# alanross/AlvaAR

Measured on NVIDIA H100. Metric: frames_per_sec_720p_1000orb_20kf_ba, higher is better.
Workload: dtype u8/f64

## Files before the change

alvaar_b200/csrc/ba.cu:

```cuda
#include "alva_common.cuh"
#include "../../include/alva_b200.h"
#include <math.h>
#include <float.h>
#include <string.h>

namespace {

constexpr int NMAX = 128;
constexpr int LIN_THREADS = 128;
constexpr int NBMAX = NMAX / 6;
constexpr int MAXKEYS = NBMAX * (NBMAX + 1) / 2;
constexpr int BS_THREADS = 128;

struct BaState {
    double radius, decrease_factor, x_cost, cand_cost, xnorm, gmax, model_change;
    double se_min, se_cur, se_ref, se_cand, se_acc_ref, se_acc_cand;
    double initial_cost, push_cost;
    int reuse_diagonal, invalid_steps, iteration, last_success, n_success, n_iter, term, done;
    int relin, step_ok, ncols, chol_ok;
    int use_gather, nb, nbad, has_last;
    int skipped, pad0;
};

struct BaProblem {
// ... 143 lines not shown
__device__ __forceinline__ double block_sum(double v, double* sm) {
    sm[threadIdx.x] = v;
    __syncthreads();
    for (int s = NT / 2; s > 0; s >>= 1) {
        if ((int)threadIdx.x < s) sm[threadIdx.x] += sm[threadIdx.x + s];
        __syncthreads();
    }
    return sm[0];
}

__device__ __forceinline__ double block_sum_dyn(double v, double* sm) {
#pragma unroll
    for (int off = 16; off; off >>= 1) v += __shfl_xor_sync(0xffffffffu, v, off);
    const int lane = threadIdx.x & 31, warp = threadIdx.x >> 5, nw = (blockDim.x + 31) >> 5;
    __syncthreads();
    if (lane == 0) sm[warp] = v;
    __syncthreads();
    if (threadIdx.x == 0) { double t = 0; for (int w = 0; w < nw; w++) t += sm[w]; sm[32] = t; }
    __syncthreads();
    return sm[32];
}
__device__ __forceinline__ double block_max_dyn(double v, double* sm) {
#pragma unroll
    for (int off = 16; off; off >>= 1) v = fmax(v, __shfl_xor_sync(0xffffffffu, v, off));
    const int lane = threadIdx.x & 31, warp = threadIdx.x >> 5, nw = (blockDim.x + 31) >> 5;
    __syncthreads();
    if (lane == 0) sm[warp] = v;
    __syncthreads();
    if (threadIdx.x == 0) { double t = sm[0]; for (int w = 1; w < nw; w++) t = fmax(t, sm[w]); sm[32] = t; }
    __syncthreads();
    return sm[32];
}

constexpr int SETUP_THREADS = 1024;
__global__ void __launch_bounds__(SETUP_THREADS) ba_setup_kernel(const BaProblem* __restrict__ probs, BaDims D) {
    const BaProblem P = probs[blockIdx.x];
    if (threadIdx.x < NBMAX) P.ga_ticket[threadIdx.x] = 0;
    __shared__ int ref[256];
    __shared__ int scan_s[SETUP_THREADS + 1];
    __shared__ int wcount[32][NBMAX + 1];
    __shared__ int run[NBMAX + 1], pl_base[NBMAX + 1];
    const int tid = threadIdx.x, lane = tid & 31, warp = tid >> 5;
    constexpr int NT = SETUP_THREADS;
    if (D.pass == 1 && (P.st->nbad == 0 || !(D.huber > 0))) {
        if (tid == 0) { P.st->done = 1; P.st->skipped = 1; P.st->use_gather = 0; P.st->has_last = 0; }
        return;
    }
    for (int k = tid; k < 256; k += NT) ref[k] = 0;
    for (int l = tid; l <= D.nlm; l += NT) P.lm_start[l] = 0;
    __syncthreads();
    for (int o = tid; o < D.nobs; o += NT) {
        const int l = P.obs_lm[o];
        if (l < 0) continue;
        atomicAdd(&P.lm_start[l + 1], 1);
        ref[P.anch_kf[l]] = 1;
        ref[P.obs_kf[o]] = 1;
    }
    __syncthreads();
    if (tid == 0) {
        int c = 0;
        for (int k = 0; k < D.nkf; k++) {
            if (!P.pose_const[k] && ref[k]) { P.pose_col[k] = c; c += 6; }
            else P.pose_col[k] = -1;
        }
        BaState& s = *P.st;
        s.ncols = c;
// ... 89 lines not shown
    maxobs = max(maxobs, __shfl_xor_sync(0xffffffffu, maxobs, 4)); maxobs = max(maxobs, __shfl_xor_sync(0xffffffffu, maxobs, 2));
    maxobs = max(maxobs, __shfl_xor_sync(0xffffffffu, maxobs, 1));
    if (lane == 0) scan_s[warp] = maxobs;
    __syncthreads();
    if (tid == 0) {
        int mo = 0;
        for (int i = 0; i < NT / 32; i++) mo = max(mo, scan_s[i]);
        P.st->use_gather = (mo < 255 && D.nlm < 65536 && D.nobs < 65535) ? 1 : 0;
    }
}

template <bool FULL>
__device__ __forceinline__ double lin_obs(const BaProblem& P, const BaDims& D, int o, int l, const double* poses, double invd_l) {
    const int ka = P.anch_kf[l], kp = P.obs_kf[o];
    double r[2], Ja[12], Jp[12], Jd[2];
    ba_evaluate(P.calib, poses + 7 * ka, poses + 7 * kp, invd_l, P.obs_uv[2 * o], P.obs_uv[2 * o + 1], P.anch_uv[2 * l],
                P.anch_uv[2 * l + 1], r, FULL ? Ja : nullptr, Jp, Jd);
    double rho0, rho1;
    huber(r[0] * r[0] + r[1] * r[1], D.huber, rho0, rho1);
    if (FULL) {
        const double sc = sqrt(rho1);
        r[0] *= sc; r[1] *= sc;
        P.res[2 * o] = r[0]; P.res[2 * o + 1] = r[1];
        Jd[0] *= sc; Jd[1] *= sc;
        P.Jd[2 * o] = Jd[0]; P.Jd[2 * o + 1] = Jd[1];
#pragma unroll
        for (int i = 0; i < 12; i++) { Ja[i] *= sc; Jp[i] *= sc; P.Ja[12 * o + i] = Ja[i]; P.Jp[12 * o + i] = Jp[i]; }
    }
    return 0.5 * rho0;
}

template <bool FULL>
__global__ void __launch_bounds__(LIN_THREADS, 7) ba_linearize_kernel(const BaProblem* __restrict__ probs, BaDims D) {
    const BaProblem P = probs[blockIdx.y];
    __shared__ double red[LIN_THREADS];
    const BaState& st = *P.st;
    const bool active = FULL ? (st.relin && !st.done) : !st.done;
    if (!active) return;
    const int o = blockIdx.x * LIN_THREADS + threadIdx.x;
    double cost = 0;
    const int l = o < D.nobs ? P.obs_lm[o] : -1;
    if (l >= 0) cost = lin_obs<FULL>(P, D, o, l, FULL ? P.poses : P.cand_poses, (FULL ? P.invd : P.cand_invd)[l]);
    const double tot = block_sum<LIN_THREADS>(cost, red);
    if (threadIdx.x == 0) P.cost_part[blockIdx.x] = tot;
}

__device__ __forceinline__ void stats_landmark(const BaProblem& P, int l) {
    double ne = 0, ge = 0;
    for (int i = P.lm_start[l]; i < P.lm_start[l + 1]; i++) {
        const int o = P.lm_obs[i];
        const double d0 = P.Jd[2 * o], d1 = P.Jd[2 * o + 1];
        ne += d0 * d0 + d1 * d1;
        ge += d0 * P.res[2 * o] + d1 * P.res[2 * o + 1];
    }
    P.ne[l] = ne;
    P.ge[l] = ge;
}
__device__ __forceinline__ void stats_pose_partial(const BaProblem& P, int b, int gt, double* v) {
    int eb = 0;
    for (int i = 0; i < b; i++) eb += P.pstart[i + 1];
    const int ee = eb + P.pstart[b + 1];
#pragma unroll
    for (int i = 0; i < 12; i++) v[i] = 0;
    for (int idx = eb + gt; idx < ee; idx += BS_THREADS) {
        const uint32_t en = P.plist[idx];
        const int l = en >> 8, su = en & 0xff;
        const int ob = P.lm_start[l];
        if (su) {
            const int o = P.lm_obs[ob + su - 1];
            const double r0 = P.res[2 * o], r1 = P.res[2 * o + 1];
#pragma unroll
            for (int c = 0; c < 6; c++) {
                const double j0 = P.Jp[12 * o + c], j1 = P.Jp[12 * o + 6 + c];
                v[c] += j0 * j0 + j1 * j1;
                v[6 + c] += j0 * r0 + j1 * r1;
            }
        } else {
            for (int i = ob; i < P.lm_start[l + 1]; i++) {
                const int o = P.lm_obs[i];
                const double r0 = P.res[2 * o], r1 = P.res[2 * o + 1];
#pragma unroll
                for (int c = 0; c < 6; c++) {
                    const double j0 = P.Ja[12 * o + c], j1 = P.Ja[12 * o + 6 + c];
                    v[c] += j0 * j0 + j1 * j1;
                    v[6 + c] += j0 * r0 + j1 * r1;
                }
            }
        }
    }
}

__global__ void __launch_bounds__(BS_THREADS) ba_stats_kernel(const BaProblem* __restrict__ probs, BaDims D) {
    const BaProblem P = probs[blockIdx.y];
    const BaState& st = *P.st;
    if (st.done || !st.relin) return;
    __shared__ double part[4][12];
    if ((int)blockIdx.x < D.nbs) {
        const int l = blockIdx.x * BS_THREADS + threadIdx.x;
        if (l >= D.nlm) return;
        stats_landmark(P, l);
        return;
    }
    const int b = blockIdx.x - D.nbs;
    if (b >= st.ncols / 6) return;
    const int lane = threadIdx.x & 31, warp = threadIdx.x >> 5;
    double v[12];
    stats_pose_partial(P, b, threadIdx.x, v);
#pragma unroll
    for (int i = 0; i < 12; i++) {
#pragma unroll
        for (int off = 16; off; off >>= 1) v[i] += __shfl_xor_sync(0xffffffffu, v[i], off);
        if (lane == 0) part[warp][i] = v[i];
    }
    __syncthreads();
    if (threadIdx.x < 12) {
        const double t = part[0][threadIdx.x] + part[1][threadIdx.x] + part[2][threadIdx.x] + part[3][threadIdx.x];
        if (threadIdx.x < 6) P.nf[6 * b + threadIdx.x] = t;
        else P.gf[6 * b + threadIdx.x - 6] = t;
    }
}

template <int MODE>
__global__ void __launch_bounds__(32) ba_pairs_kernel(const BaProblem* __restrict__ probs, BaDims D) {
    const BaProblem P = probs[blockIdx.y];
    BaState& st = *P.st;
// ... 122 lines not shown
    __syncthreads();
    if (tid == 0) {
        if (st.last_success) st.n_success++;
        st.n_iter++;
        int cont = 1;
        if (st.iteration >= D.max_iter) { st.term = 1; cont = 0; }
        else if (st.last_success && st.gmax <= 1e-10) { st.term = 0; cont = 0; }
        else if (st.radius <= 1e-32) { st.term = 0; cont = 0; }
        if (!cont) st.done = 1;
        else { st.iteration++; st.last_success = 0; }
        go = cont;
    }
    __syncthreads();
    if (!go) return;
    const bool reuse = st.reuse_diagonal;
    const double radius = st.radius;
    __syncthreads();
    for (int i = tid; i < n; i += NT) {
        if (!reuse) P.diagf[i] = fmin(fmax(P.nf[i] * P.scf[i] * P.scf[i], 1e-6), 1e32);
        P.Df[i] = sqrt(P.diagf[i] / radius);
    }
    for (int l = tid; l < D.nlm; l += NT) {
        if (!reuse) P.diage[l] = fmin(fmax(P.ne[l] * P.sce[l] * P.sce[l], 1e-6), 1e32);
        P.De[l] = sqrt(P.diage[l] / radius);
    }
    for (int i = tid; i < NMAX * NMAX; i += NT) P.S[i] = 0;
    for (int i = tid; i < NMAX; i += NT) P.rhs[i] = 0;
    __syncthreads();
    for (int i = tid; i < n; i += NT) P.S[i * NMAX + i] = P.Df[i] * P.Df[i];
    if (tid == 0) st.reuse_diagonal = 1;
}

__global__ void __launch_bounds__(CT_THREADS) ba_pre_kernel(const BaProblem* __restrict__ probs, BaDims D) {
    const BaProblem P = probs[blockIdx.x];
    ba_pre_body(P, D);
}

template <bool DENSE>
__device__ void schur_landmark(const BaProblem& P, const BaDims& D, int l) {
    if (DENSE) {
        double* row = P.Wt + (size_t)l * NMAX;
        for (int i = 0; i < NMAX; i++) row[i] = 0.0;
    }
    if (l >= D.nlm) return;
    const int b = P.lm_start[l], e = P.lm_start[l + 1];
    if (e == b) return;
    const int ca = P.pose_col[P.anch_kf[l]];
    const double sce = P.sce[l];
    double ete = P.De[l] * P.De[l], etb = 0, wa[6] = {0, 0, 0, 0, 0, 0};
    double sca[6];
    for (int c = 0; c < 6; c++) sca[c] = ca >= 0 ? P.scf[ca + c] : 0.0;
    double Saa[36];
    for (int i = 0; i < 36; i++) Saa[i] = 0;
    double rha[6] = {0, 0, 0, 0, 0, 0};
    for (int i = b; i < e; i++) {
        const int o = P.lm_obs[i];
        const int cp = P.pose_col[P.obs_kf[o]];
        const double e0 = P.Jd[2 * o] * sce, e1 = P.Jd[2 * o + 1] * sce;
        const double r0 = P.res[2 * o], r1 = P.res[2 * o + 1];
        ete += e0 * e0 + e1 * e1;
        etb += e0 * r0 + e1 * r1;
        double Fa[12], Fp[12];
        for (int c = 0; c < 6; c++) {
            Fa[c] = P.Ja[12 * o + c] * sca[c]; Fa[6 + c] = P.Ja[12 * o + 6 + c] * sca[c];
            const double s = cp >= 0 ? P.scf[cp + c] : 0.0;
            Fp[c] = P.Jp[12 * o + c] * s; Fp[6 + c] = P.Jp[12 * o + 6 + c] * s;
// ... 41 lines not shown
            for (int c = 0; c < 6; c++) {
                row[ci + c] += P.wp[6 * oi + c] * rs;
                atomicAdd(&P.rhs[ci + c], -P.wp[6 * oi + c] * inv * etb);
            }
        }
        return;
    }
    for (int i = b; i < e; i++) {
        const int oi = P.lm_obs[i];
        const int ci = P.pose_col[P.obs_kf[oi]];
        if (ci < 0) continue;
        double wi[6];
        for (int c = 0; c < 6; c++) wi[c] = P.wp[6 * oi + c];
        for (int a = 0; a < 6; a++) atomicAdd(&P.rhs[ci + a], -wi[a] * inv * etb);
        if (ca >= 0)
            for (int a = 0; a < 6; a++)
                for (int c = 0; c < 6; c++) {
                    const double x = -wa[a] * inv * wi[c];
                    atomicAdd(&P.S[(ca + a) * NMAX + ci + c], x);
                    atomicAdd(&P.S[(ci + c) * NMAX + ca + a], x);
                }
        for (int j = b; j < e; j++) {
            const int oj = P.lm_obs[j];
            const int cj = P.pose_col[P.obs_kf[oj]];
            if (cj < 0) continue;
            for (int a = 0; a < 6; a++)
                for (int c = 0; c < 6; c++) atomicAdd(&P.S[(ci + a) * NMAX + cj + c], -wi[a] * inv * P.wp[6 * oj + c]);
        }
    }
}

template <bool DENSE>
__global__ void __launch_bounds__(128) ba_schur_kernel(const BaProblem* __restrict__ probs, BaDims D) {
    const BaProblem P = probs[blockIdx.y];
    if (P.st->done) return;
    if (!DENSE && P.st->use_gather) return;
    const int l = blockIdx.x * 128 + threadIdx.x;
    if (l >= D.nlm_pad) return;
    schur_landmark<DENSE>(P, D, l);
}

__device__ __forceinline__ void dmma_m8n8k4(double& c0, double& c1, double a, double b) {
    asm volatile("mma.sync.aligned.m8n8k4.row.col.f64.f64.f64.f64 {%0, %1}, {%2}, {%3}, {%0, %1};"
                 : "+d"(c0), "+d"(c1)
                 : "d"(a), "d"(b));
}

constexpr int SYRK_KSPLIT = 8;

__global__ void __launch_bounds__(128) ba_syrk_dmma_kernel(const BaProblem* __restrict__ probs, BaDims D) {
    const BaProblem P = probs[blockIdx.z];
    if (P.st->done) return;
    __shared__ double part[4][32][33];
    const int lane = threadIdx.x & 31, warp = threadIdx.x >> 5;
    const int bi = blockIdx.x >> 2, bj = blockIdx.x & 3;
    const int i0 = bi * 32, j0 = bj * 32;
    const int n = P.st->ncols;
    if (i0 >= n || j0 >= n) return;
    const int ksteps = D.nlm_pad / 4;
    const int per = (ksteps + SYRK_KSPLIT - 1) / SYRK_KSPLIT;
    const int kb = blockIdx.y * per, ke = min(ksteps, kb + per);
    double acc[4][4][2];
#pragma unroll
    for (int a = 0; a < 4; a++)
#pragma unroll
        for (int b = 0; b < 4; b++) acc[a][b][0] = acc[a][b][1] = 0.0;
    const int kr = lane & 3, cc = lane >> 2;
    for (int ks = kb + warp; ks < ke; ks += 4) {
        const double* row = P.Wt + (size_t)(4 * ks + kr) * NMAX;
        double av[4], bv[4];
#pragma unroll
        for (int t = 0; t < 4; t++) { av[t] = __ldg(row + i0 + 8 * t + cc); bv[t] = __ldg(row + j0 + 8 * t + cc); }
#pragma unroll
        for (int a = 0; a < 4; a++)
#pragma unroll
            for (int b = 0; b < 4; b++) dmma_m8n8k4(acc[a][b][0], acc[a][b][1], av[a], bv[b]);
    }
#pragma unroll
    for (int a = 0; a < 4; a++)
#pragma unroll
        for (int b = 0; b < 4; b++) {
            part[warp][8 * a + cc][8 * b + 2 * kr] = acc[a][b][0];
            part[warp][8 * a + cc][8 * b + 2 * kr + 1] = acc[a][b][1];
        }
    __syncthreads();
    for (int t = threadIdx.x; t < 32 * 32; t += 128) {
        const int r = t >> 5, c = t & 31;
        const double v = part[0][r][c] + part[1][r][c] + part[2][r][c] + part[3][r][c];
        if (v != 0.0) atomicAdd(&P.S[(i0 + r) * NMAX + j0 + c], -v);
    }
}


__device__ __forceinline__ void lm_landmark(const BaProblem& P, int l) {
    const int b = P.lm_start[l], e = P.lm_start[l + 1];
    if (e == b) return;
    const int ca = P.pose_col[P.anch_kf[l]];
    const double sce = P.sce[l];
    double ete = P.De[l] * P.De[l], etb = 0, wa[6] = {0, 0, 0, 0, 0, 0};
    for (int i = b; i < e; i++) {
        const int o = P.lm_obs[i];
        const int cp = P.pose_col[P.obs_kf[o]];
        const double e0 = P.Jd[2 * o] * sce, e1 = P.Jd[2 * o + 1] * sce;
        ete += e0 * e0 + e1 * e1;
        etb += e0 * P.res[2 * o] + e1 * P.res[2 * o + 1];
        for (int c = 0; c < 6; c++) {
            if (ca >= 0) wa[c] += (e0 * P.Ja[12 * o + c] + e1 * P.Ja[12 * o + 6 + c]) * P.scf[ca + c];
            P.wp[6 * o + c] = cp >= 0 ? (e0 * P.Jp[12 * o + c] + e1 * P.Jp[12 * o + 6 + c]) * P.scf[cp + c] : 0.0;
        }
    }
    P.ete[l] = ete;
    P.etb[l] = etb;
    for (int c = 0; c < 6; c++) P.wa[6 * l + c] = wa[c];
}
__global__ void __launch_bounds__(128) ba_lm_kernel(const BaProblem* __restrict__ probs, BaDims D) {
    const BaProblem P = probs[blockIdx.y];
    if (P.st->done) return;
    const int l = blockIdx.x * 128 + threadIdx.x;
    if (P.st->use_gather) { if (l < D.nlm) lm_landmark(P, l); }
    else if (l < D.nlm) schur_landmark<false>(P, D, l);
}

template <bool TRANSPOSE>
__device__ __forceinline__ void gather_entry(const BaProblem& P, uint64_t en, const double* sci, const double* scj, double* acc,
                                             double* rh) {
    const int l = (int)(en >> 48), su = (int)(en >> 40) & 0xff, sv = (int)(en >> 32) & 0xff;
    const double inv = 1.0 / P.ete[l], etb = P.etb[l];
    const int ou = su ? (int)(en >> 16) & 0xffff : -1, ov = sv ? (int)en & 0xffff : -1;
    double wu[6], wv[6];
#pragma unroll
    for (int c = 0; c < 6; c++) {
        wu[c] = (su ? P.wp[6 * ou + c] : P.wa[6 * l + c]) * inv;
        wv[c] = sv ? P.wp[6 * ov + c] : P.wa[6 * l + c];
    }
#define ACC(a, c) acc[TRANSPOSE ? 6 * (c) + (a) : 6 * (a) + (c)]
#pragma unroll
    for (int a = 0; a < 6; a++)
#pragma unroll
        for (int c = 0; c < 6; c++) ACC(a, c) -= wu[a] * wv[c];
    if (su == 0 && sv == 0) {
        const int ob = P.lm_start[l], oe = P.lm_start[l + 1];
        for (int i = ob; i < oe; i++) {
            const int o = P.lm_obs[i];
            double F0[6], F1[6];
#pragma unroll
            for (int c = 0; c < 6; c++) { F0[c] = P.Ja[12 * o + c] * sci[c]; F1[c] = P.Ja[12 * o + 6 + c] * sci[c]; }
            const double r0 = P.res[2 * o], r1 = P.res[2 * o + 1];
#pragma unroll
// ... 9 lines not shown
    } else if (su == sv) {
        double F0[6], F1[6];
#pragma unroll
        for (int c = 0; c < 6; c++) { F0[c] = P.Jp[12 * ou + c] * sci[c]; F1[c] = P.Jp[12 * ou + 6 + c] * sci[c]; }
        const double r0 = P.res[2 * ou], r1 = P.res[2 * ou + 1];
#pragma unroll
        for (int a = 0; a < 6; a++) {
            if (!TRANSPOSE) rh[a] += F0[a] * r0 + F1[a] * r1 - wu[a] * etb;
#pragma unroll
            for (int c = 0; c < 6; c++) ACC(a, c) += F0[a] * F0[c] + F1[a] * F1[c];
        }
    } else if (su == 0 || sv == 0) {
        const int o = su ? ou : ov;
        double A0[6], A1[6];
#pragma unroll
        for (int a = 0; a < 6; a++) {
            A0[a] = (su ? P.Jp[12 * o + a] : P.Ja[12 * o + a]) * sci[a];
            A1[a] = (su ? P.Jp[12 * o + 6 + a] : P.Ja[12 * o + 6 + a]) * sci[a];
        }
#pragma unroll
        for (int c = 0; c < 6; c++) {
            const double b0 = (sv ? P.Jp[12 * o + c] : P.Ja[12 * o + c]) * scj[c];
            const double b1 = (sv ? P.Jp[12 * o + 6 + c] : P.Ja[12 * o + 6 + c]) * scj[c];
#pragma unroll
            for (int a = 0; a < 6; a++) ACC(a, c) += A0[a] * b0 + A1[a] * b1;
        }
    }
#undef ACC
}

constexpr int GA_THREADS = 64, GA_SPLIT = 8;
constexpr int GA_GRID = NBMAX * GA_SPLIT + (MAXKEYS - NBMAX);
__global__ void __launch_bounds__(GA_THREADS, 8) ba_gather_kernel(const BaProblem* __restrict__ probs, BaDims D) {
    const BaProblem P = probs[blockIdx.y];
    const BaState& st = *P.st;
    if (st.done || !st.use_gather) return;
    int bi, bj, part = 0, nparts = 1;
    if ((int)blockIdx.x < NBMAX * GA_SPLIT) { bi = bj = blockIdx.x / GA_SPLIT; part = blockIdx.x % GA_SPLIT; nparts = GA_SPLIT; }
    else {
        int rem = blockIdx.x - NBMAX * GA_SPLIT;
        bi = 0;
        while (bi < NBMAX - 1 && rem >= NBMAX - 1 - bi) { rem -= NBMAX - 1 - bi; bi++; }
        bj = bi + 1 + rem;
    }
    if (bi >= st.nb || bj >= st.nb) return;
    const int blk = bi * NBMAX + bj;
    __shared__ double red[GA_THREADS / 32][42];
    __shared__ int last_s;
    const int tid = threadIdx.x, lane = tid & 31, warp = tid >> 5;
    const int ci = 6 * bi, cj = 6 * bj;
    const int eb = P.blk_off[blk], ee = eb + P.blk_start[blk + 1];
    double acc[36], rh[6];
#pragma unroll
    for (int i = 0; i < 36; i++) acc[i] = 0.0;
#pragma unroll
    for (int i = 0; i < 6; i++) rh[i] = 0.0;
    double sci[6], scj[6];
#pragma unroll
    for (int c = 0; c < 6; c++) { sci[c] = P.scf[ci + c]; scj[c] = P.scf[cj + c]; }
    for (int idx = eb + part * GA_THREADS + tid; idx < ee; idx += nparts * GA_THREADS) {
        const uint64_t en = P.pairs[idx];
        gather_entry<false>(P, en, sci, scj, acc, rh);
    }
#pragma unroll
    for (int i = 0; i < 36; i++) {
#pragma unroll
// ... 109 lines not shown
        }
    }
    if (tile) {
#pragma unroll
        for (int r = 0; r < 4; r++)
#pragma unroll
            for (int c = 0; c < 4; c++) {
                const int gr = r0 + r, gc = c0 + c;
                if (gr <= n && gc < n) V[gr * ld + gc] = a[r][c];
            }
    }
    __syncthreads();
    if (tid < 32) {
        double xr[4];
#pragma unroll
        for (int q = 0; q < 4; q++) { const int i = lane + 32 * q; xr[q] = i < n ? V[n * ld + i] * invd[i] : 0.0; }
        for (int i = n - 1; i >= 0; i--) {
            const int qi = i >> 5;
            const double own = qi == 0 ? xr[0] : qi == 1 ? xr[1] : qi == 2 ? xr[2] : xr[3];
            const double xi = __shfl_sync(0xffffffffu, own, i & 31);
#pragma unroll
            for (int q = 0; q < 4; q++) {
                const int k = lane + 32 * q;
                if (k < i) xr[q] -= V[i * ld + k] * invd[k] * xi;
            }
        }
#pragma unroll
        for (int q = 0; q < 4; q++) { const int i = lane + 32 * q; if (i < n) P.yf[i] = xr[q]; }
        if (lane == 0) st.chol_ok = ok_s;
    }
}
__global__ void __launch_bounds__(CH_THREADS) ba_chol_kernel(const BaProblem* __restrict__ probs, BaDims D) {
    extern __shared__ double sm[];
    const BaProblem P = probs[blockIdx.x];
    if (P.st->done) return;
    ba_chol_body(P, sm);
}

__device__ __forceinline__ void backsub_cand_pose(const BaProblem& P, int k, double* out) {
    const int c0 = P.pose_col[k];
    if (c0 >= 0) {
        double dlt[6];
        for (int i = 0; i < 6; i++) dlt[i] = -P.yf[c0 + i] * P.scf[c0 + i];
        se3_plus(P.poses + 7 * k, dlt, out);
    } else
        for (int i = 0; i < 7; i++) out[i] = P.poses[7 * k + i];
}
__device__ __forceinline__ double backsub_landmark(const BaProblem& P, int l) {
    const int b = P.lm_start[l], e = P.lm_start[l + 1];
    double ye = 0, acc = 0;
    if (e > b) {
        double s = P.etb[l];
        const int ca = P.pose_col[P.anch_kf[l]];
        if (ca >= 0) for (int c = 0; c < 6; c++) s -= P.wa[6 * l + c] * P.yf[ca + c];
        for (int i = b; i < e; i++) {
            const int o = P.lm_obs[i];
            const int cp = P.pose_col[P.obs_kf[o]];
            if (cp >= 0) for (int c = 0; c < 6; c++) s -= P.wp[6 * o + c] * P.yf[cp + c];
        }
        ye = s / P.ete[l];
        const double se = -ye * P.sce[l];
        for (int i = b; i < e; i++) {
            const int o = P.lm_obs[i];
            const int cp = P.pose_col[P.obs_kf[o]];
            double m0 = P.Jd[2 * o] * se, m1 = P.Jd[2 * o + 1] * se;
            for (int c = 0; c < 6; c++) {
                if (ca >= 0) { const double q = -P.yf[ca + c] * P.scf[ca + c]; m0 += P.Ja[12 * o + c] * q; m1 += P.Ja[12 * o + 6 + c] * q; }
                if (cp >= 0) { const double q = -P.yf[cp + c] * P.scf[cp + c]; m0 += P.Jp[12 * o + c] * q; m1 += P.Jp[12 * o + 6 + c] * q; }
            }
            acc += m0 * (P.res[2 * o] + m0 / 2.0) + m1 * (P.res[2 * o + 1] + m1 / 2.0);
        }
        P.cand_invd[l] = P.invd[l] + se;
    } else
        P.cand_invd[l] = P.invd[l];
    P.ye[l] = ye;
    return acc;
}
__global__ void __launch_bounds__(BS_THREADS) ba_backsub_kernel(const BaProblem* __restrict__ probs, BaDims D) {
    const BaProblem P = probs[blockIdx.y];
    __shared__ double red[BS_THREADS];
    if (P.st->done) return;
    const int l = blockIdx.x * BS_THREADS + threadIdx.x;
    if (blockIdx.x == 0 && (int)threadIdx.x < D.nkf) backsub_cand_pose(P, threadIdx.x, P.cand_poses + 7 * threadIdx.x);
    const double acc = l < D.nlm ? backsub_landmark(P, l) : 0.0;
    const double tot = block_sum<BS_THREADS>(acc, red);
    if (threadIdx.x == 0) P.mc_part[blockIdx.x] = tot;
}

__device__ void ba_post_body(const BaProblem& P, const BaDims& D) {
    BaState& st = *P.st;
    __shared__ double red[34];
    __shared__ int accept_s;
    const int tid = threadIdx.x, NT = blockDim.x;
    if (st.done) return;
    double mcs = 0;
    for (int i = tid; i < D.nbs; i += NT) mcs += P.mc_part[i];
    const double model_change = -block_sum_dyn(mcs, red);
    const bool valid = st.chol_ok && (model_change > 0.0);
    __syncthreads();
    if (!valid) {
        if (tid == 0) {
            st.model_change = model_change;
            if (++st.invalid_steps >= 5) { st.term = 2; st.done = 1; }
            st.radius *= 0.5;
            st.reuse_diagonal = 1;
            st.push_cost = st.x_cost;
            st.chol_ok = 1;
        }
        return;
    }
    if (P.last_poses) {
// ... 25 lines not shown
            const double hist = (st.se_ref - cand_cost) / (st.se_acc_ref + mc);
            const double quality = fmax(rel, hist);
            if (quality > 1e-3) {
                accept = 1;
                st.radius = fmin(1e16, st.radius / fmax(1.0 / 3.0, 1.0 - pow(2.0 * quality - 1.0, 3)));
                st.decrease_factor = 2.0;
                st.reuse_diagonal = 0;
                st.se_cur = cand_cost; st.se_acc_cand += mc; st.se_acc_ref += mc;
                bool nonmono = false;
                if (st.se_cur < st.se_min) { st.se_min = st.se_cur; st.se_cand = st.se_cur; st.se_acc_cand = 0; }
                else { nonmono = true; if (st.se_cur > st.se_cand) { st.se_cand = st.se_cur; st.se_acc_cand = 0; } }
                if (!nonmono) { st.se_ref = st.se_cand; st.se_acc_ref = st.se_acc_cand; }
                st.last_success = 1;
                st.relin = 1;
            } else {
                st.radius = st.radius / st.decrease_factor;
                st.decrease_factor *= 2.0;
                st.reuse_diagonal = 1;
                st.push_cost = cand_cost;
            }
        }
        accept_s = accept;
    }
    __syncthreads();
    if (accept_s) {
        for (int i = tid; i < 7 * D.nkf; i += NT) P.poses[i] = P.cand_poses[i];
        for (int l = tid; l < D.nlm; l += NT) P.invd[l] = P.cand_invd[l];
        for (int i = tid; i < NMAX; i += NT) { P.nf[i] = 0; P.gf[i] = 0; }
        for (int l = tid; l < D.nlm; l += NT) { P.ne[l] = 0; P.ge[l] = 0; }
    }
}

__global__ void __launch_bounds__(CT_THREADS) ba_post_kernel(const BaProblem* __restrict__ probs, BaDims D) {
    const BaProblem P = probs[blockIdx.x];
    ba_post_body(P, D);
}

__global__ void ba_linearize_dump_kernel(const double* calib, const double* poses, const double* invd, const int32_t* anch_kf,
                                         const double* anch_uv, const int32_t* obs_kf, const int32_t* obs_lm,
                                         const double* obs_uv, int nobs, double hub, double* res, double* Ja, double* Jp,
                                         double* Jd, double* cost) {
    const int o = blockIdx.x * blockDim.x + threadIdx.x;
    if (o >= nobs) return;
    const int l = obs_lm[o];
    double r[2] = {0, 0}, A[12], Pp[12], Dd[2];
    for (int i = 0; i < 12; i++) A[i] = Pp[i] = 0;
    Dd[0] = Dd[1] = 0;
    double c = 0;
    if (l >= 0) {
        ba_evaluate(calib, poses + 7 * anch_kf[l], poses + 7 * obs_kf[o], invd[l], obs_uv[2 * o], obs_uv[2 * o + 1],
                    anch_uv[2 * l], anch_uv[2 * l + 1], r, A, Pp, Dd);
        double rho0, rho1;
        huber(r[0] * r[0] + r[1] * r[1], hub, rho0, rho1);
        c = 0.5 * rho0;
        const double sc = sqrt(rho1);
        r[0] *= sc; r[1] *= sc; Dd[0] *= sc; Dd[1] *= sc;
        for (int i = 0; i < 12; i++) { A[i] *= sc; Pp[i] *= sc; }
    }
    res[2 * o] = r[0]; res[2 * o + 1] = r[1]; Jd[2 * o] = Dd[0]; Jd[2 * o + 1] = Dd[1];
    for (int i = 0; i < 12; i++) { Ja[12 * o + i] = A[i]; Jp[12 * o + i] = Pp[i]; }
    cost[o] = c;
}

__global__ void ba_local_init_kernel(const BaProblem* __restrict__ probs, BaDims D) {
    const BaProblem P = probs[blockIdx.y];
    const int o = blockIdx.x * blockDim.x + threadIdx.x;
    if (o < D.nobs) { P.obs_lm_w[o] = P.obs_lm_in[o]; P.flags[o] = 0; }
    if (o == 0) { P.st->nbad = 0; P.st->has_last = 0; P.st->skipped = 0; }
}

template <int MARK>
__global__ void __launch_bounds__(LIN_THREADS) ba_flag_kernel(const BaProblem* __restrict__ probs, BaDims D, double chi2_thr) {
    const BaProblem P = probs[blockIdx.y];
    BaState& st = *P.st;
    if (MARK == 2 && st.skipped) return;
    const int o = blockIdx.x * LIN_THREADS + threadIdx.x;
    const int l = o < D.nobs ? P.obs_lm_w[o] : -1;
    if (l < 0) return;
    const double* poses = st.has_last ? P.last_poses : P.poses;
    const double* invd = st.has_last ? P.last_invd : P.invd;
    double r[2];
    const bool front = ba_evaluate(P.calib, poses + 7 * P.anch_kf[l], poses + 7 * P.obs_kf[o], invd[l], P.obs_uv[2 * o],
                                   P.obs_uv[2 * o + 1], P.anch_uv[2 * l], P.anch_uv[2 * l + 1], r, nullptr, nullptr, nullptr);
    if (r[0] * r[0] + r[1] * r[1] > chi2_thr || !front) {
        P.flags[o] = MARK;
        if (MARK == 1) { P.obs_lm_w[o] = -1; atomicAdd(&st.nbad, 1); }
    }
}

__global__ void ba_summary_local_kernel(const BaProblem* __restrict__ probs, double* __restrict__ summary, int second) {
    const BaState& st = *probs[blockIdx.x].st;
    if (threadIdx.x == 0) {
        double* s = summary + 10 * blockIdx.x + 5 * second;
        if (second && st.skipped) { s[0] = s[1] = s[2] = s[3] = s[4] = 0; return; }
        s[0] = st.initial_cost; s[1] = st.x_cost; s[2] = st.n_success; s[3] = st.n_iter; s[4] = st.term;
    }
}

__global__ void ba_summary_kernel(const BaProblem* __restrict__ probs, double* __restrict__ summary) {
    const BaState& st = *probs[blockIdx.x].st;
    if (threadIdx.x == 0) {
        double* s = summary + 8 * blockIdx.x;
        s[0] = st.initial_cost; s[1] = st.x_cost; s[2] = st.n_success; s[3] = st.n_iter; s[4] = st.term;
        s[5] = st.ncols; s[6] = st.radius; s[7] = st.iteration;
    }
}

size_t align_up(size_t v, size_t a) { return (v + a - 1) / a * a; }

}

static int g_ba_dense_schur = 0;
static int g_ba_ctl_threads = CT_THREADS;

static size_t ba_ws_bytes(int nkf, int nlm, int nobs, int nblk) {
    size_t d = 0;
    if (g_ba_dense_schur) d += (size_t)((nlm + 3) / 4 * 4) * NMAX;
    d += (size_t)nobs * (2 + 12 + 12 + 2 + 6);
    d += 5 * (size_t)NMAX;
    d += 5 * (size_t)nlm;
    d += (size_t)nlm * (1 + 1 + 6 + 1);
    d += (size_t)NMAX * NMAX + 2 * NMAX;
    d += (size_t)nkf * 7 + nlm;
    d += (size_t)nblk;
    d += (size_t)((nlm + BS_THREADS - 1) / BS_THREADS);
    d += (size_t)NBMAX * GA_SPLIT * 42;
    size_t bytes = d * sizeof(double);
    bytes += align_up((size_t)nkf * 4, 8) + align_up((size_t)(nlm + 1) * 4, 8) + align_up((size_t)nobs * 4, 8);
    bytes += align_up((size_t)nobs * 4, 8) + align_up((size_t)nlm * 4, 8);
    bytes += align_up((size_t)(NBMAX + 1) * 4, 8) + align_up(((size_t)nobs + (size_t)nlm) * 4, 8);
    bytes += 2 * align_up((size_t)(NBMAX * NBMAX + 1) * 4, 8) + align_up((size_t)(8 * (size_t)nobs + 2 * (size_t)nlm) * 8, 8);
    bytes += align_up((size_t)NBMAX * 4, 8);
// ... 45 lines not shown
            P.ga_part = take((size_t)NBMAX * GA_SPLIT * 42);
            P.last_poses = local ? take(7 * (size_t)nkf) : nullptr;
            P.last_invd = local ? take(nlm) : nullptr;
            uint8_t* b = reinterpret_cast<uint8_t*>(d);
            P.pose_col = reinterpret_cast<int32_t*>(b); b += align_up((size_t)nkf * 4, 8);
            P.lm_start = reinterpret_cast<int32_t*>(b); b += align_up((size_t)(nlm + 1) * 4, 8);
            P.lm_obs = reinterpret_cast<int32_t*>(b); b += align_up((size_t)nobs * 4, 8);
            P.obs_col = reinterpret_cast<int32_t*>(b); b += align_up((size_t)nobs * 4, 8);
            P.anch_col = reinterpret_cast<int32_t*>(b); b += align_up((size_t)nlm * 4, 8);
            P.pstart = reinterpret_cast<int32_t*>(b); b += align_up((size_t)(NBMAX + 1) * 4, 8);
            P.plist = reinterpret_cast<uint32_t*>(b); b += align_up(((size_t)nobs + (size_t)nlm) * 4, 8);
            P.blk_start = reinterpret_cast<int32_t*>(b); b += align_up((size_t)(NBMAX * NBMAX + 1) * 4, 8);
            P.blk_off = reinterpret_cast<int32_t*>(b); b += align_up((size_t)(NBMAX * NBMAX + 1) * 4, 8);
            P.pairs = reinterpret_cast<uint64_t*>(b); b += align_up((size_t)(8 * (size_t)nobs + 2 * (size_t)nlm) * 8, 8);
            P.ga_ticket = reinterpret_cast<int32_t*>(b); b += align_up((size_t)NBMAX * 4, 8);
            P.obs_lm_in = nullptr; P.obs_lm_w = nullptr; P.flags = nullptr;
            if (local) {
                P.obs_lm_in = P.obs_lm;
                P.obs_lm_w = reinterpret_cast<int32_t*>(b); b += align_up((size_t)nobs * 4, 8);
                P.obs_lm = P.obs_lm_w;
                P.flags = flags + (size_t)nobs * p;
            }
            P.st = reinterpret_cast<BaState*>(b);
        }
        ALVA_CUDA(cudaMemcpyAsync(ws, hp, sizeof(BaProblem) * nprob, cudaMemcpyHostToDevice, ctx->stream));
        ALVA_CUDA(cudaStreamSynchronize(ctx->stream));
        ctx->ba_table_key = key;
    }
    *dp_out = reinterpret_cast<const BaProblem*>(ws);
    *D_out = BaDims{nkf, nlm, nobs, nblk, 0.0, 0, (nlm + 3) / 4 * 4, 8 * nobs + 2 * nlm, (nlm + BS_THREADS - 1) / BS_THREADS, 0};
    return 0;
}

static int ba_run_solve(alva_ctx* ctx, const BaProblem* dp, const BaDims& D, int nprob) {
    const bool dense = g_ba_dense_schur != 0;
    const size_t chol_smem = ((size_t)NMAX * (NMAX + 1) + NMAX) * sizeof(double);
    ALVA_CUDA(cudaFuncSetAttribute(ba_chol_kernel, cudaFuncAttributeMaxDynamicSharedMemorySize, (int)chol_smem));
    ba_setup_kernel<<<nprob, SETUP_THREADS, 0, ctx->stream>>>(dp, D);
    ALVA_LAUNCH_CHECK(ctx);
    const dim3 lin_grid(D.nblk, nprob), schur_grid((D.nlm_pad + 127) / 128, nprob), syrk_grid(16, SYRK_KSPLIT, nprob);
    const dim3 key_grid(GA_GRID, nprob), bs_grid(D.nbs, nprob), stats_grid(D.nbs + NBMAX, nprob);
    bool forked = false;
    if (!dense) {
        const dim3 pr_grid(NBMAX, nprob);
        cudaStream_t ps = ctx->stream;
        if (ctx->aux_stream && cudaEventRecord(ctx->aux_fork, ctx->stream) == cudaSuccess &&
            cudaStreamWaitEvent(ctx->aux_stream, ctx->aux_fork, 0) == cudaSuccess) { ps = ctx->aux_stream; forked = true; }
        ba_pairs_kernel<0><<<pr_grid, 32, 0, ps>>>(dp, D);
        ALVA_LAUNCH_CHECK(ctx);
        ba_pairs_kernel<1><<<pr_grid, 32, 0, ps>>>(dp, D);
        ALVA_LAUNCH_CHECK(ctx);
        if (forked) ALVA_CUDA(cudaEventRecord(ctx->aux_join, ps));
    }
    for (int it = 0; it <= D.max_iter; it++) {
        ba_linearize_kernel<true><<<lin_grid, LIN_THREADS, 0, ctx->stream>>>(dp, D);
        ALVA_LAUNCH_CHECK(ctx);
        ba_stats_kernel<<<stats_grid, BS_THREADS, 0, ctx->stream>>>(dp, D);
        ALVA_LAUNCH_CHECK(ctx);
        ba_pre_kernel<<<nprob, g_ba_ctl_threads, 0, ctx->stream>>>(dp, D);
        ALVA_LAUNCH_CHECK(ctx);
        if (it == D.max_iter) {
            if (forked) { ALVA_CUDA(cudaStreamWaitEvent(ctx->stream, ctx->aux_join, 0)); forked = false; }
            break;
        }
        if (dense) {
            ba_schur_kernel<true><<<schur_grid, 128, 0, ctx->stream>>>(dp, D);
            ALVA_LAUNCH_CHECK(ctx);
            ba_syrk_dmma_kernel<<<syrk_grid, 128, 0, ctx->stream>>>(dp, D);
            ALVA_LAUNCH_CHECK(ctx);
        } else {
            if (forked) { ALVA_CUDA(cudaStreamWaitEvent(ctx->stream, ctx->aux_join, 0)); forked = false; }
            ba_lm_kernel<<<schur_grid, 128, 0, ctx->stream>>>(dp, D);
            ALVA_LAUNCH_CHECK(ctx);
            ba_gather_kernel<<<key_grid, GA_THREADS, 0, ctx->stream>>>(dp, D);
            ALVA_LAUNCH_CHECK(ctx);
        }
        ba_chol_kernel<<<nprob, CH_THREADS, chol_smem, ctx->stream>>>(dp, D);
        ALVA_LAUNCH_CHECK(ctx);
        ba_backsub_kernel<<<bs_grid, BS_THREADS, 0, ctx->stream>>>(dp, D);
        ALVA_LAUNCH_CHECK(ctx);
        ba_linearize_kernel<false><<<lin_grid, LIN_THREADS, 0, ctx->stream>>>(dp, D);
        ALVA_LAUNCH_CHECK(ctx);
        ba_post_kernel<<<nprob, g_ba_ctl_threads, 0, ctx->stream>>>(dp, D);
        ALVA_LAUNCH_CHECK(ctx);
    }
    return 0;
}

static bool ba_args_ok(alva_ctx* ctx, int nprob, int nkf, int nlm, int nobs, const void* calib, const void* poses,
                       const void* pose_const, const void* invd, const void* anch_kf, const void* anch_uv, const void* obs_kf,
                       const void* obs_lm, const void* obs_uv, int max_iter) {
    return ctx && nprob >= 1 && nkf >= 1 && nkf <= 256 && nlm >= 1 && nobs >= 1 && calib && poses && pose_const && invd &&
           anch_kf && anch_uv && obs_kf && obs_lm && obs_uv && max_iter >= 0;
}

extern "C" int alva_k_ba_solve(alva_ctx* ctx, int nprob, int nkf, int nlm, int nobs, const double* calib, double* poses,
                               const uint8_t* pose_const, double* invd, const int32_t* anch_kf, const double* anch_uv,
                               const int32_t* obs_kf, const int32_t* obs_lm, const double* obs_uv, double huber_delta,
                               int max_iter, double* summary) { AlvaDeviceGuard guard__(ctx);
    if (!ba_args_ok(ctx, nprob, nkf, nlm, nobs, calib, poses, pose_const, invd, anch_kf, anch_uv, obs_kf, obs_lm, obs_uv, max_iter)) {
        alva_set_error("alva_k_ba_solve: bad argument (need 1 <= nkf <= 256)");
        return ALVA_E_INVALID;
    }
    const BaProblem* dp;
    BaDims D;
    if (int e = ba_prepare(ctx, nprob, nkf, nlm, nobs, calib, poses, pose_const, invd, anch_kf, anch_uv, obs_kf, obs_lm, obs_uv,
                           nullptr, &dp, &D))
        return e;
    D.huber = huber_delta; D.max_iter = max_iter;
    if (int e = ba_run_solve(ctx, dp, D, nprob)) return e;
    if (summary) {
        ba_summary_kernel<<<nprob, 32, 0, ctx->stream>>>(dp, summary);
        ALVA_LAUNCH_CHECK(ctx);
    }
    return 0;
}

extern "C" int alva_k_ba_local(alva_ctx* ctx, int nprob, int nkf, int nlm, int nobs, const double* calib, double* poses,
                               const uint8_t* pose_const, double* invd, const int32_t* anch_kf, const double* anch_uv,
                               const int32_t* obs_kf, const int32_t* obs_lm, const double* obs_uv, double huber_delta,
                               double chi2_thr, int max_iter, int32_t* flags, double* summary) { AlvaDeviceGuard guard__(ctx);
    if (!ba_args_ok(ctx, nprob, nkf, nlm, nobs, calib, poses, pose_const, invd, anch_kf, anch_uv, obs_kf, obs_lm, obs_uv, max_iter) ||
        !flags) {
        alva_set_error("alva_k_ba_local: bad argument (need 1 <= nkf <= 256, flags != NULL)");
        return ALVA_E_INVALID;
    }
    const BaProblem* dp;
    BaDims D;
    if (int e = ba_prepare(ctx, nprob, nkf, nlm, nobs, calib, poses, pose_const, invd, anch_kf, anch_uv, obs_kf, obs_lm, obs_uv,
                           flags, &dp, &D))
        return e;
    D.huber = huber_delta; D.max_iter = max_iter;
    const dim3 obs_grid(D.nblk, nprob);
    ba_local_init_kernel<<<obs_grid, LIN_THREADS, 0, ctx->stream>>>(dp, D);
    ALVA_LAUNCH_CHECK(ctx);
    if (int e = ba_run_solve(ctx, dp, D, nprob)) return e;
    if (summary) { ba_summary_local_kernel<<<nprob, 32, 0, ctx->stream>>>(dp, summary, 0); ALVA_LAUNCH_CHECK(ctx); }
    ba_flag_kernel<1><<<obs_grid, LIN_THREADS, 0, ctx->stream>>>(dp, D, chi2_thr);
    ALVA_LAUNCH_CHECK(ctx);
    D.pass = 1; D.max_iter = 5;
    if (int e = ba_run_solve(ctx, dp, D, nprob)) return e;
    ba_flag_kernel<2><<<obs_grid, LIN_THREADS, 0, ctx->stream>>>(dp, D, chi2_thr);
    ALVA_LAUNCH_CHECK(ctx);
    if (summary) { ba_summary_local_kernel<<<nprob, 32, 0, ctx->stream>>>(dp, summary, 1); ALVA_LAUNCH_CHECK(ctx); }
    return 0;
}
// ... 40 lines not shown
```

Measured before the change: 36540.

## Chain BA solver kernels with programmatic dependent launch

Every kernel in the bundle-adjustment LM loop now starts with griddepcontrol.wait, and the host launches them through cudaLaunchKernelEx with the programmatic stream serialization attribute. This lets the next kernel's launch and block scheduling overlap the tail of the previous kernel, cutting the launch gaps between the many small kernels in each iteration. The iteration body is also moved into helper functions. Kernels never trigger early, so each one still waits for its predecessor to complete fully, and the benefit is limited to hiding launch latency. Cross-stream event waits turn off PDL on the next launch.

```diff
diff --git a/alvaar_b200/csrc/ba.cu b/alvaar_b200/csrc/ba.cu
--- a/alvaar_b200/csrc/ba.cu
+++ b/alvaar_b200/csrc/ba.cu
@@ -199,6 +199,8 @@
     return sm[32];
 }
 
+__device__ __forceinline__ void chain_wait() { asm volatile("griddepcontrol.wait;" ::: "memory"); }
+
 constexpr int SETUP_THREADS = 1024;
 __global__ void __launch_bounds__(SETUP_THREADS) ba_setup_kernel(const BaProblem* __restrict__ probs, BaDims D) {
     const BaProblem P = probs[blockIdx.x];
@@ -354,6 +356,7 @@
 
 template <bool FULL>
 __global__ void __launch_bounds__(LIN_THREADS, 7) ba_linearize_kernel(const BaProblem* __restrict__ probs, BaDims D) {
+    chain_wait();
     const BaProblem P = probs[blockIdx.y];
     __shared__ double red[LIN_THREADS];
     const BaState& st = *P.st;
@@ -413,6 +416,7 @@
 }
 
 __global__ void __launch_bounds__(BS_THREADS) ba_stats_kernel(const BaProblem* __restrict__ probs, BaDims D) {
+    chain_wait();
     const BaProblem P = probs[blockIdx.y];
     const BaState& st = *P.st;
     if (st.done || !st.relin) return;
@@ -601,6 +605,7 @@
 }
 
 __global__ void __launch_bounds__(CT_THREADS) ba_pre_kernel(const BaProblem* __restrict__ probs, BaDims D) {
+    chain_wait();
     const BaProblem P = probs[blockIdx.x];
     ba_pre_body(P, D);
 }
@@ -708,6 +713,7 @@
 
 template <bool DENSE>
 __global__ void __launch_bounds__(128) ba_schur_kernel(const BaProblem* __restrict__ probs, BaDims D) {
+    chain_wait();
     const BaProblem P = probs[blockIdx.y];
     if (P.st->done) return;
     if (!DENSE && P.st->use_gather) return;
@@ -725,6 +731,7 @@
 constexpr int SYRK_KSPLIT = 8;
 
 __global__ void __launch_bounds__(128) ba_syrk_dmma_kernel(const BaProblem* __restrict__ probs, BaDims D) {
+    chain_wait();
     const BaProblem P = probs[blockIdx.z];
     if (P.st->done) return;
     __shared__ double part[4][32][33];
@@ -790,6 +797,7 @@
     for (int c = 0; c < 6; c++) P.wa[6 * l + c] = wa[c];
 }
 __global__ void __launch_bounds__(128) ba_lm_kernel(const BaProblem* __restrict__ probs, BaDims D) {
+    chain_wait();
     const BaProblem P = probs[blockIdx.y];
     if (P.st->done) return;
     const int l = blockIdx.x * 128 + threadIdx.x;
@@ -865,6 +873,7 @@
 constexpr int GA_THREADS = 64, GA_SPLIT = 8;
 constexpr int GA_GRID = NBMAX * GA_SPLIT + (MAXKEYS - NBMAX);
 __global__ void __launch_bounds__(GA_THREADS, 8) ba_gather_kernel(const BaProblem* __restrict__ probs, BaDims D) {
+    chain_wait();
     const BaProblem P = probs[blockIdx.y];
     const BaState& st = *P.st;
     if (st.done || !st.use_gather) return;
@@ -1040,6 +1049,7 @@
 }
 __global__ void __launch_bounds__(CH_THREADS) ba_chol_kernel(const BaProblem* __restrict__ probs, BaDims D) {
     extern __shared__ double sm[];
+    chain_wait();
     const BaProblem P = probs[blockIdx.x];
     if (P.st->done) return;
     ba_chol_body(P, sm);
@@ -1085,6 +1095,7 @@
     return acc;
 }
 __global__ void __launch_bounds__(BS_THREADS) ba_backsub_kernel(const BaProblem* __restrict__ probs, BaDims D) {
+    chain_wait();
     const BaProblem P = probs[blockIdx.y];
     __shared__ double red[BS_THREADS];
     if (P.st->done) return;
@@ -1176,6 +1187,7 @@
 }
 
 __global__ void __launch_bounds__(CT_THREADS) ba_post_kernel(const BaProblem* __restrict__ probs, BaDims D) {
+    chain_wait();
     const BaProblem P = probs[blockIdx.x];
     ba_post_body(P, D);
 }
@@ -1242,6 +1254,7 @@
 }
 
 __global__ void ba_summary_kernel(const BaProblem* __restrict__ probs, double* __restrict__ summary) {
+    chain_wait();
     const BaState& st = *probs[blockIdx.x].st;
     if (threadIdx.x == 0) {
         double* s = summary + 8 * blockIdx.x;
@@ -1353,19 +1366,53 @@
     return 0;
 }
 
+template <class... K, class... A>
+static cudaError_t ba_launch(cudaStream_t s, bool pdl, void (*kernel)(K...), dim3 grid, dim3 block, size_t smem, A... args) {
+    cudaLaunchAttribute at[1];
+    at[0].id = cudaLaunchAttributeProgrammaticStreamSerialization;
+    at[0].val.programmaticStreamSerializationAllowed = 1;
+    cudaLaunchConfig_t cfg = {};
+    cfg.gridDim = grid; cfg.blockDim = block; cfg.dynamicSmemBytes = smem; cfg.stream = s;
+    cfg.attrs = at; cfg.numAttrs = pdl ? 1 : 0;
+    return cudaLaunchKernelEx(&cfg, kernel, args...);
+}
+#define BA_LAUNCH(...) do { ALVA_CUDA(ba_launch(__VA_ARGS__)); ctx->launches++; } while (0)
+
+static int ba_linearize_pass(alva_ctx* ctx, cudaStream_t s, const BaProblem* dp, const BaDims& D, int nprob, bool pdl) {
+    BA_LAUNCH(s, pdl, ba_linearize_kernel<true>, dim3(D.nblk, nprob), dim3(LIN_THREADS), 0, dp, D);
+    BA_LAUNCH(s, true, ba_stats_kernel, dim3(D.nbs + NBMAX, nprob), dim3(BS_THREADS), 0, dp, D);
+    BA_LAUNCH(s, true, ba_pre_kernel, dim3(nprob), dim3(g_ba_ctl_threads), 0, dp, D);
+    return 0;
+}
+
+static int ba_iteration(alva_ctx* ctx, cudaStream_t s, const BaProblem* dp, const BaDims& D, int nprob, bool join) {
+    const size_t chol_smem = ((size_t)NMAX * (NMAX + 1) + NMAX) * sizeof(double);
+    if (int e = ba_linearize_pass(ctx, s, dp, D, nprob, true)) return e;
+    if (g_ba_dense_schur) {
+        BA_LAUNCH(s, true, ba_schur_kernel<true>, dim3((D.nlm_pad + 127) / 128, nprob), dim3(128), 0, dp, D);
+        BA_LAUNCH(s, true, ba_syrk_dmma_kernel, dim3(16, SYRK_KSPLIT, nprob), dim3(128), 0, dp, D);
+    } else {
+        if (join) ALVA_CUDA(cudaStreamWaitEvent(s, ctx->aux_join, 0));
+        BA_LAUNCH(s, !join, ba_lm_kernel, dim3((D.nlm_pad + 127) / 128, nprob), dim3(128), 0, dp, D);
+        BA_LAUNCH(s, true, ba_gather_kernel, dim3(GA_GRID, nprob), dim3(GA_THREADS), 0, dp, D);
+    }
+    BA_LAUNCH(s, true, ba_chol_kernel, dim3(nprob), dim3(CH_THREADS), chol_smem, dp, D);
+    BA_LAUNCH(s, true, ba_backsub_kernel, dim3(D.nbs, nprob), dim3(BS_THREADS), 0, dp, D);
+    BA_LAUNCH(s, true, ba_linearize_kernel<false>, dim3(D.nblk, nprob), dim3(LIN_THREADS), 0, dp, D);
+    BA_LAUNCH(s, true, ba_post_kernel, dim3(nprob), dim3(g_ba_ctl_threads), 0, dp, D);
+    return 0;
+}
+
 static int ba_run_solve(alva_ctx* ctx, const BaProblem* dp, const BaDims& D, int nprob) {
-    const bool dense = g_ba_dense_schur != 0;
     const size_t chol_smem = ((size_t)NMAX * (NMAX + 1) + NMAX) * sizeof(double);
     ALVA_CUDA(cudaFuncSetAttribute(ba_chol_kernel, cudaFuncAttributeMaxDynamicSharedMemorySize, (int)chol_smem));
-    ba_setup_kernel<<<nprob, SETUP_THREADS, 0, ctx->stream>>>(dp, D);
-    ALVA_LAUNCH_CHECK(ctx);
-    const dim3 lin_grid(D.nblk, nprob), schur_grid((D.nlm_pad + 127) / 128, nprob), syrk_grid(16, SYRK_KSPLIT, nprob);
-    const dim3 key_grid(GA_GRID, nprob), bs_grid(D.nbs, nprob), stats_grid(D.nbs + NBMAX, nprob);
+    cudaStream_t st = ctx->stream;
+    BA_LAUNCH(st, false, ba_setup_kernel, dim3(nprob), dim3(SETUP_THREADS), 0, dp, D);
     bool forked = false;
-    if (!dense) {
+    if (!g_ba_dense_schur) {
         const dim3 pr_grid(NBMAX, nprob);
-        cudaStream_t ps = ctx->stream;
-        if (ctx->aux_stream && cudaEventRecord(ctx->aux_fork, ctx->stream) == cudaSuccess &&
+        cudaStream_t ps = st;
+        if (ctx->aux_stream && cudaEventRecord(ctx->aux_fork, st) == cudaSuccess &&
             cudaStreamWaitEvent(ctx->aux_stream, ctx->aux_fork, 0) == cudaSuccess) { ps = ctx->aux_stream; forked = true; }
         ba_pairs_kernel<0><<<pr_grid, 32, 0, ps>>>(dp, D);
         ALVA_LAUNCH_CHECK(ctx);
@@ -1373,39 +1420,12 @@
         ALVA_LAUNCH_CHECK(ctx);
         if (forked) ALVA_CUDA(cudaEventRecord(ctx->aux_join, ps));
     }
-    for (int it = 0; it <= D.max_iter; it++) {
-        ba_linearize_kernel<true><<<lin_grid, LIN_THREADS, 0, ctx->stream>>>(dp, D);
-        ALVA_LAUNCH_CHECK(ctx);
-        ba_stats_kernel<<<stats_grid, BS_THREADS, 0, ctx->stream>>>(dp, D);
-        ALVA_LAUNCH_CHECK(ctx);
-        ba_pre_kernel<<<nprob, g_ba_ctl_threads, 0, ctx->stream>>>(dp, D);
-        ALVA_LAUNCH_CHECK(ctx);
-        if (it == D.max_iter) {
-            if (forked) { ALVA_CUDA(cudaStreamWaitEvent(ctx->stream, ctx->aux_join, 0)); forked = false; }
-            break;
-        }
-        if (dense) {
-            ba_schur_kernel<true><<<schur_grid, 128, 0, ctx->stream>>>(dp, D);
-            ALVA_LAUNCH_CHECK(ctx);
-            ba_syrk_dmma_kernel<<<syrk_grid, 128, 0, ctx->stream>>>(dp, D);
-            ALVA_LAUNCH_CHECK(ctx);
-        } else {
-            if (forked) { ALVA_CUDA(cudaStreamWaitEvent(ctx->stream, ctx->aux_join, 0)); forked = false; }
-            ba_lm_kernel<<<schur_grid, 128, 0, ctx->stream>>>(dp, D);
-            ALVA_LAUNCH_CHECK(ctx);
-            ba_gather_kernel<<<key_grid, GA_THREADS, 0, ctx->stream>>>(dp, D);
-            ALVA_LAUNCH_CHECK(ctx);
-        }
-        ba_chol_kernel<<<nprob, CH_THREADS, chol_smem, ctx->stream>>>(dp, D);
-        ALVA_LAUNCH_CHECK(ctx);
-        ba_backsub_kernel<<<bs_grid, BS_THREADS, 0, ctx->stream>>>(dp, D);
-        ALVA_LAUNCH_CHECK(ctx);
-        ba_linearize_kernel<false><<<lin_grid, LIN_THREADS, 0, ctx->stream>>>(dp, D);
-        ALVA_LAUNCH_CHECK(ctx);
-        ba_post_kernel<<<nprob, g_ba_ctl_threads, 0, ctx->stream>>>(dp, D);
-        ALVA_LAUNCH_CHECK(ctx);
-    }
-    return 0;
+    for (int it = 0; it < D.max_iter; it++) {
+        if (int e = ba_iteration(ctx, st, dp, D, nprob, forked)) return e;
+        forked = false;
+    }
+    if (forked) ALVA_CUDA(cudaStreamWaitEvent(st, ctx->aux_join, 0));
+    return ba_linearize_pass(ctx, st, dp, D, nprob, !forked);
 }
 
 static bool ba_args_ok(alva_ctx* ctx, int nprob, int nkf, int nlm, int nobs, const void* calib, const void* poses,
@@ -1431,8 +1451,7 @@
     D.huber = huber_delta; D.max_iter = max_iter;
     if (int e = ba_run_solve(ctx, dp, D, nprob)) return e;
     if (summary) {
-        ba_summary_kernel<<<nprob, 32, 0, ctx->stream>>>(dp, summary);
-        ALVA_LAUNCH_CHECK(ctx);
+        BA_LAUNCH(ctx->stream, true, ba_summary_kernel, dim3(nprob), dim3(32), 0, dp, summary);
     }
     return 0;
 }
```

Result: no change. 36620 (median of 6 runs) (+0.2%).
